# megvii-research/CVPR2023-UniDistill

Hardware: AMD Instinct MI355X
Metric: distill-train samples/sec (nuScenes frame); bev_pool+voxelize HBM GB/s (higher is better)
Workload: dtype f32; 1 GPU; camera_exp_distill_lidar: student+teacher distillation step, 6 cams 256x704, 30000-pt cloud, 40 GT boxes, fwd+bwd+AdamW; batch_per_gpu=4, global_batch=4, parallelism=dp1, layout=channels-last dense convs, executor=eager+DDP, strict_no_library_fallthrough=True, wgrad_stream=on, ranks=1, dist_backend=none (single process)

## Files before the change

cvpr2023-unidistill_amd/csrc/spconv_conv.hip:

```cpp
#include "ud_common.h"
#include "ud_prof.h"
#include "spconv_tile.h"
#include <cstdlib>

namespace {

template <int CIN_P, int COUT_P>
__global__ __launch_bounds__(256) void k_conv_mfma(const float* __restrict__ in, int cin,
                                                   const int32_t* __restrict__ nbr, int K,
                                                   int mirror, const float* __restrict__ W,
                                                   WStrides ws, const float* __restrict__ bias,
                                                   float* __restrict__ out, int cout, int Mout) {
  constexpr int LDA = CIN_P + 4;
  extern __shared__ __attribute__((aligned(16))) char smem[];
  float* As = reinterpret_cast<float*>(smem);
  float* Bs = As + kTM * LDA;
  int* s_nbr = reinterpret_cast<int*>(Bs + COUT_P * LDA);
  const int tid = threadIdx.x, lane = tid & 63, wave = tid >> 6;
  const int g = lane >> 4, li = lane & 15;
  const int row0 = blockIdx.x * kTM;
  constexpr int NT = COUT_P / 16;
  f32x4 acc[NT];
#pragma unroll
  for (int t = 0; t < NT; ++t) acc[t] = (f32x4){0.f, 0.f, 0.f, 0.f};
// ... 57 lines not shown
    __syncthreads();
  }
#pragma unroll
  for (int t = 0; t < NT; ++t) {
    const int col = t * 16 + li;
    if (col >= cout) continue;
    const float bv = bias ? bias[col] : 0.f;
#pragma unroll
    for (int r = 0; r < 4; ++r) {
      const int row = row0 + wave * 16 + 4 * g + r;
      if (row < Mout) out[(size_t)row * cout + col] = acc[t][r] + bv;
    }
  }
}


template <int CIN_P, int COUT_P, bool VA, bool VB>
__global__ __launch_bounds__(512) void k_conv_mfma_v2(const float* __restrict__ in, int cin,
                                                      const int32_t* __restrict__ nbr, int K,
                                                      int mirror, const float* __restrict__ W,
                                                      WStrides ws, const float* __restrict__ bias,
                                                      float* __restrict__ out, int cout, int Mout,
                                                      const int32_t* __restrict__ order,
                                                      ConvEpilogue ep) {
  constexpr int LDA = CIN_P + 8;
  constexpr int NT = COUT_P / 16;
  constexpr int A4 = kTM2 * (CIN_P / 4) / 512;
  constexpr int B4 = (COUT_P * (CIN_P / 4) + 511) / 512;
  constexpr int BU = COUT_P * (CIN_P / 4);
  extern __shared__ __attribute__((aligned(16))) char smem[];
  float* As = reinterpret_cast<float*>(smem);
  float* Bs = As + kTM2 * LDA;
  int* s_nbr = reinterpret_cast<int*>(Bs + COUT_P * LDA);
  unsigned& s_active = *reinterpret_cast<unsigned*>(s_nbr + K * kTM2);
  int* s_row = s_nbr + K * kTM2 + 4;
  const int tid = threadIdx.x, lane = tid & 63, wave = tid >> 6;
  const int g = lane >> 4, li = lane & 15;
  const SpTile tile = sp_tile_setup<16>(s_nbr, s_active, s_row, nbr, K, mirror, order, Mout, tid, lane, wave);
  const unsigned active = tile.active, wmask = tile.wmask;
  f32x4 acc[NT];
#pragma unroll
  for (int t = 0; t < NT; ++t) acc[t] = (f32x4){0.f, 0.f, 0.f, 0.f};
  float4 ra[A4], rb[VB ? B4 : 1];
  constexpr int PER = CIN_P / 4, RPP = 512 / PER;
  const int r0 = tid / PER, c4 = (tid % PER) * 4;
  const bool cok = c4 < cin;
  const float* in_c = in + (cok ? c4 : 0);
  const int wc4 = cok ? c4 : 0;

  auto fetch_a = [&](int k, int j) {
    const int rr = s_nbr[k * kTM2 + r0 + RPP * j];
    if constexpr (VA) {
      ra[j] = *reinterpret_cast<const float4*>(in_c + (size_t)(rr < 0 ? 0 : rr) * cin);
    } else {
      float4 v = make_float4(0.f, 0.f, 0.f, 0.f);
      if (rr >= 0) {
        const float* src = in + (size_t)rr * cin + c4;
        if (c4 + 0 < cin) v.x = src[0];
        if (c4 + 1 < cin) v.y = src[1];
        if (c4 + 2 < cin) v.z = src[2];
        if (c4 + 3 < cin) v.w = src[3];
// ... 108 lines not shown
__global__ __launch_bounds__(512) void k_conv_mfma_bf16(const float* __restrict__ in, int cin,
                                                        const int32_t* __restrict__ nbr, int K,
                                                        int mirror, const float* __restrict__ W,
                                                        WStrides ws, const float* __restrict__ bias,
                                                        float* __restrict__ out, int cout, int Mout,
                                                        const int32_t* __restrict__ order,
                                                        ConvEpilogue ep, int io) {
  const bool in_bf = io & 1, out_bf = io & 2, w_bf = io & 4;
  const unsigned short* in_h = reinterpret_cast<const unsigned short*>(in);
  const unsigned short* W_h = reinterpret_cast<const unsigned short*>(W);
  constexpr int LDB = CIN_P + 8;
  constexpr int NT = COUT_P / 16;
  constexpr int A4 = kTM2 * (CIN_P / 4) / 512;
  constexpr int B4 = (COUT_P * (CIN_P / 4) + 511) / 512;
  constexpr int BU = COUT_P * (CIN_P / 4);
  extern __shared__ __attribute__((aligned(16))) char smem[];
  unsigned short* As = reinterpret_cast<unsigned short*>(smem);
  unsigned short* Bs = As + kTM2 * LDB;
  int* s_nbr = reinterpret_cast<int*>(Bs + COUT_P * LDB);
  unsigned& s_active = *reinterpret_cast<unsigned*>(s_nbr + K * kTM2);
  int* s_row = s_nbr + K * kTM2 + 4;
  const int tid = threadIdx.x, lane = tid & 63, wave = tid >> 6;
  const int g = lane >> 4, li = lane & 15;
  const SpTile tile = sp_tile_setup<16>(s_nbr, s_active, s_row, nbr, K, mirror, order, Mout, tid, lane, wave);
  const unsigned active = tile.active, wmask = tile.wmask;
  f32x4 acc[NT];
#pragma unroll
  for (int t = 0; t < NT; ++t) acc[t] = (f32x4){0.f, 0.f, 0.f, 0.f};
  const bool vecA = (cin & 3) == 0;
  const bool vecB = (ws.sc == 1) && vecA;
  float4 ra[A4];
  auto fetch = [&](int k) {
#pragma unroll
    for (int j = 0; j < A4; ++j) {
      const int u = tid + 512 * j;
      const int row = u / (CIN_P / 4), c4 = (u - row * (CIN_P / 4)) * 4;
      const int rr = s_nbr[k * kTM2 + row];
      float4 v = make_float4(0.f, 0.f, 0.f, 0.f);
      if (rr >= 0 && in_bf) {
        if (c4 < cin) {
          const uint2 h = *reinterpret_cast<const uint2*>(in_h + (size_t)rr * cin + c4);
          v.x = __uint_as_float(h.x);
          v.y = __uint_as_float(h.y);
        }
      } else if (rr >= 0) {
        const float* src = in + (size_t)rr * cin + c4;
        if (vecA) {
// ... 88 lines not shown
  return ((a > o ? a : o) + 15) / 16 * 16;
}

template <int CIN_P, int COUT_P>
__global__ __launch_bounds__(512) void k_conv_mfma_bf16_fast(
    const unsigned short* __restrict__ in, int cin, const int32_t* __restrict__ nbr, int K, int mirror,
    const unsigned short* __restrict__ W, WStrides ws, const float* __restrict__ bias,
    unsigned short* __restrict__ out, int cout, int Mout, const int32_t* __restrict__ order,
    ConvEpilogue ep) {
  constexpr int LDB = CIN_P + 8;
  constexpr int NT = COUT_P / 16;
  constexpr int AU = kTM2 * (CIN_P / 8);
  constexpr int BU = COUT_P * (CIN_P / 8);
  constexpr int A8 = (AU + 511) / 512, B8 = (BU + 511) / 512;
  extern __shared__ __attribute__((aligned(16))) char smem[];
  unsigned short* As = reinterpret_cast<unsigned short*>(smem);
  unsigned short* Bs = As + kTM2 * LDB;
  int* s_nbr = reinterpret_cast<int*>(smem + fast_front_bytes(CIN_P, COUT_P));
  unsigned& s_active = *reinterpret_cast<unsigned*>(s_nbr + K * kTM2);
  int* s_row = s_nbr + K * kTM2 + 4;
  float* Os = reinterpret_cast<float*>(smem);
  const int tid = threadIdx.x, lane = tid & 63, wave = tid >> 6;
  const int g = lane >> 4, li = lane & 15;
  const SpTile tile = sp_tile_setup<16>(s_nbr, s_active, s_row, nbr, K, mirror, order, Mout, tid, lane, wave);
  const unsigned active = tile.active, wmask = tile.wmask;
  f32x4 acc[NT];
#pragma unroll
  for (int t = 0; t < NT; ++t) acc[t] = (f32x4){0.f, 0.f, 0.f, 0.f};
  uint4 ra[A8], rb[B8];
  auto fetch = [&](int k) {
#pragma unroll
    for (int j = 0; j < A8; ++j) {
      const int u = tid + 512 * j;
      ra[j] = make_uint4(0u, 0u, 0u, 0u);
      if (u < AU) {
        const int row = u / (CIN_P / 8), c8 = (u - row * (CIN_P / 8)) * 8;
        const int rr = s_nbr[k * kTM2 + row];
        if (rr >= 0 && c8 < cin) ra[j] = *reinterpret_cast<const uint4*>(in + (size_t)rr * cin + c8);
      }
    }
#pragma unroll
    for (int j = 0; j < B8; ++j) {
      const int u = tid + 512 * j;
      rb[j] = make_uint4(0u, 0u, 0u, 0u);
      if (u < BU) {
        const int n = u / (CIN_P / 8), c8 = (u - n * (CIN_P / 8)) * 8;
        if (n < cout && c8 < cin) rb[j] = *reinterpret_cast<const uint4*>(W + n * ws.sn + k * ws.sk + c8);
// ... 53 lines not shown
  const size_t o = (size_t)kTM2 * (cout_p + 4) * 4;
  return ((a > o ? a : o) + 15) / 16 * 16;
}

template <int CIN_P, int COUT_P>
__global__ __launch_bounds__(512) void k_conv_mfma_bf16_dma(
    const unsigned short* __restrict__ in, int cin, const int32_t* __restrict__ nbr, int K, int mirror,
    const unsigned short* __restrict__ W, WStrides ws, const float* __restrict__ bias,
    unsigned short* __restrict__ out, int cout, int Mout, const int32_t* __restrict__ order,
    ConvEpilogue ep) {
  constexpr int NT = COUT_P / 16;
  constexpr int S = CIN_P / 8;
  constexpr int RPP = 64 / S;
  constexpr int APIECES = kTM2 / RPP, BPIECES = (COUT_P + RPP - 1) / RPP;
  extern __shared__ __attribute__((aligned(16))) char smem[];
  unsigned short* As = reinterpret_cast<unsigned short*>(smem);
  unsigned short* Bs = As + 2 * kTM2 * CIN_P;
  int* s_nbr = reinterpret_cast<int*>(smem + dma_front_bytes(CIN_P, COUT_P));
  unsigned& s_active = *reinterpret_cast<unsigned*>(s_nbr + K * kTM2);
  int* s_row = s_nbr + K * kTM2 + 4;
  float* Os = reinterpret_cast<float*>(smem);
  const int tid = threadIdx.x, lane = tid & 63, wave = tid >> 6;
  const int g = lane >> 4, li = lane & 15;
  const SpTile tile = sp_tile_setup<16>(s_nbr, s_active, s_row, nbr, K, mirror, order, Mout, tid, lane, wave);
  const unsigned active = tile.active, wmask = tile.wmask;
  f32x4 acc[NT];
#pragma unroll
  for (int t = 0; t < NT; ++t) acc[t] = (f32x4){0.f, 0.f, 0.f, 0.f};
  auto swz = [](int r) -> int {
    if (S == 16) return r & 15;
    if (S == 8) return (r >> 1) & 7;
    const int q = (r >> 2) & 3;
    return q == 0 ? 0 : (q == 1 ? 2 : (q == 2 ? 3 : 1));
  };
  const unsigned short* zero = reinterpret_cast<const unsigned short*>(g_sp_zero16);
  const int prow = lane / S, pslot = lane % S;
  auto stage = [&](int k, int buf) {
#pragma unroll
    for (int j = 0; j < (APIECES + 7) / 8; ++j) {
      const int piece = wave + 8 * j;
      if (piece < APIECES) {
        const int r = piece * RPP + prow;
        const int rr = s_nbr[k * kTM2 + r];
        const unsigned short* src = rr >= 0 ? in + (size_t)rr * cin + ((pslot ^ swz(r)) << 3) : zero;
        __builtin_amdgcn_global_load_lds((const __attribute__((address_space(1))) void*)src,
                                         (__attribute__((address_space(3))) void*)(As + (buf * kTM2 + piece * RPP) * CIN_P),
                                         16, 0, 0);
// ... 53 lines not shown
  const long long t = (long long)blockIdx.x * 256 + threadIdx.x;
  if (t >= (long long)Mout * cout) return;
  const int row = (int)(t / cout), n = (int)(t - (long long)row * cout);
  float acc = 0.f;
  for (int k = 0; k < K; ++k) {
    const int r = nbr[(size_t)row * K + (mirror ? K - 1 - k : k)];
    if (r < 0) continue;
    const float* x = in + (size_t)r * cin;
    const float* w = W + n * ws.sn + k * ws.sk;
    for (int c = 0; c < cin; ++c) acc = fmaf(x[c], w[c * ws.sc], acc);
  }
  out[t] = acc + (bias ? bias[n] : 0.f);
}

constexpr unsigned kDmaOob = 0xFFFF0000u;
__device__ __forceinline__ void sp_dma16(__amdgpu_buffer_rsrc_t rsrc, unsigned voff, unsigned soff, unsigned lds_wave_base) {
  __builtin_amdgcn_raw_ptr_buffer_load_lds(rsrc, (__attribute__((address_space(3))) void*)(size_t)lds_wave_base, 16, voff, soff, 0, 0);
}

template <int CIN, int COUT, int NBUF>
__global__ __launch_bounds__(512) void k_conv_dma_f32(const float* __restrict__ in, const int32_t* __restrict__ nbr, int K,
                                                      int mirror, const float* __restrict__ W, WStrides ws,
                                                      const float* __restrict__ bias, float* __restrict__ out, int Mout,
                                                      const int32_t* __restrict__ order, ConvEpilogue ep) {
  constexpr int NT = COUT / 32;
  constexpr int kAB = kTM2 * 256, kWB = COUT * 256, kStage = kAB + kWB;
  constexpr int kHalves = CIN / 64;
  constexpr int kAPieces = kTM2 / 4, kWPieces = COUT / 4;
  extern __shared__ __attribute__((aligned(16))) char smem[];
  int* s_nbr = reinterpret_cast<int*>(smem + NBUF * kStage);
  unsigned& s_active = *reinterpret_cast<unsigned*>(s_nbr + K * kTM2);
  int* s_row = s_nbr + K * kTM2 + 4;
  const int tid = threadIdx.x, lane = tid & 63;
  const int wave = __builtin_amdgcn_readfirstlane(tid >> 6);
  const int g = lane >> 4, li = lane & 15;
  const int wm = wave >> 1, wn = wave & 1;
  const SpTile tile = sp_tile_setup<32>(s_nbr, s_active, s_row, nbr, K, mirror, order, Mout, tid, lane, wm);
  const unsigned active = tile.active, wmask = tile.wmask;
  f32x4 acc[2][NT];
#pragma unroll
  for (int i = 0; i < 2; ++i)
#pragma unroll
    for (int t = 0; t < NT; ++t) acc[i][t] = (f32x4){0.f, 0.f, 0.f, 0.f};

  const __amdgpu_buffer_rsrc_t rin = __builtin_amdgcn_make_buffer_rsrc((void*)in, 0, (int)kDmaOob, 0x00020000);
  const __amdgpu_buffer_rsrc_t rw = __builtin_amdgcn_make_buffer_rsrc((void*)W, 0, (int)kDmaOob, 0x00020000);
  const unsigned swz = (unsigned)((li ^ ((4 * wave + g) & 15)) << 4);
  unsigned wvo[kWPieces / 8];
#pragma unroll
  for (int i = 0; i < kWPieces / 8; ++i) wvo[i] = (unsigned)(4 * (wave + 8 * i) + g) * (unsigned)ws.sn * 4u + swz;
  auto stage = [&](int k, int half, int buf) {
    const unsigned sb = (unsigned)(size_t)smem + buf * kStage;
    int rr[kAPieces / 8];
    {
      const unsigned na = NBUF * kStage + (unsigned)(k * kTM2 + 4 * wave + g) * 4u;
#pragma unroll
      for (int i = 0; i < kAPieces / 8; ++i) asm volatile("ds_read_b32 %0, %1 offset:%2" : "=v"(rr[i]) : "v"(na), "n"(i * 128));
      asm volatile("s_waitcnt lgkmcnt(0)" ::: "memory");
#pragma unroll
      for (int i = 0; i < kAPieces / 8; ++i) asm volatile("" : "+v"(rr[i]));
// ... 82 lines not shown
  for (int t = 0; t < NT; ++t) {
    const int col = wn * (COUT / 2) + t * 16 + li;
    const float bv = bias ? bias[col] : 0.f;
    const float sc = ep.scale ? ep.scale[col] : 1.f;
    const float sh = ep.shift ? ep.shift[col] : 0.f;
#pragma unroll
    for (int i = 0; i < 2; ++i)
#pragma unroll
      for (int r = 0; r < 4; ++r) {
        const int row = s_row[wm * 32 + 16 * i + 4 * g + r];
        if (row >= 0) {
          float v = acc[i][t][r] + bv;
          if (ep.scale) v = v * sc + sh;
          if (ep.residual) v += ep.residual[(size_t)row * COUT + col];
          if (ep.relu) v = fmaxf(v, 0.f);
          out[(size_t)row * COUT + col] = v;
        }
      }
  }
}

template <int CIN, int COUT>
int launch_conv_dma_f32(const float* in, const int32_t* nbr, int K, int mirror, const float* W, WStrides ws,
                        const float* bias, float* out, int Mout, const int32_t* order, ConvEpilogue ep,
                        hipStream_t stream) {
  constexpr int NBUF = 2;
  constexpr size_t front = NBUF * (size_t)(kTM2 * 256 + COUT * 256);
  const size_t lds = front + sp_tile_meta_bytes(K);
  if (lds > kSpLdsMax) return UD_ERR_UNSUPPORTED;
  static UdDeviceOnce attr_set;
  if (const int e = ud_allow_dyn_lds(attr_set, sp_lds_limit(front), k_conv_dma_f32<CIN, COUT, NBUF>)) return e;
  k_conv_dma_f32<CIN, COUT, NBUF><<<ud_div_up(Mout, kTM2), 512, lds, stream>>>(in, nbr, K, mirror, W, ws, bias, out, Mout, order, ep);
  UD_LAUNCH_CHECK();
  return UD_OK;
}

template <int CIN_P, int COUT_P>
int launch_conv_v2(const float* in, int cin, const int32_t* nbr, int K, int mirror, const float* W,
                   WStrides ws, const float* bias, float* out, int cout, int Mout,
                   const int32_t* order, ConvEpilogue ep, hipStream_t stream) {
  constexpr size_t front = (size_t)(kTM2 + COUT_P) * (CIN_P + 8) * sizeof(float);
  const size_t lds = front + sp_tile_meta_bytes(K);
  static UdDeviceOnce attr_set;
  if (const int e = ud_allow_dyn_lds(attr_set, sp_lds_limit(front), k_conv_mfma_v2<CIN_P, COUT_P, true, true>,
                                     k_conv_mfma_v2<CIN_P, COUT_P, true, false>, k_conv_mfma_v2<CIN_P, COUT_P, false, false>))
    return e;
  const bool va = (cin & 3) == 0, vb = va && ws.sc == 1;
  const dim3 grid(ud_div_up(Mout, kTM2));
  if (vb)
    k_conv_mfma_v2<CIN_P, COUT_P, true, true><<<grid, 512, lds, stream>>>(in, cin, nbr, K, mirror, W, ws, bias, out, cout,
                                                                          Mout, order, ep);
  else if (va)
    k_conv_mfma_v2<CIN_P, COUT_P, true, false><<<grid, 512, lds, stream>>>(in, cin, nbr, K, mirror, W, ws, bias, out, cout,
                                                                           Mout, order, ep);
  else
    k_conv_mfma_v2<CIN_P, COUT_P, false, false><<<grid, 512, lds, stream>>>(in, cin, nbr, K, mirror, W, ws, bias, out,
                                                                            cout, Mout, order, ep);
  UD_LAUNCH_CHECK();
  return UD_OK;
}

template <int CIN_P, int COUT_P>
int launch_conv_bf16(const float* in, int cin, const int32_t* nbr, int K, int mirror, const float* W,
                     WStrides ws, const float* bias, float* out, int cout, int Mout,
                     const int32_t* order, ConvEpilogue ep, int io, hipStream_t stream) {
  constexpr int CP = CIN_P < 32 ? 32 : CIN_P;
  if ((io & 1) && (cin & 3)) return UD_ERR_UNSUPPORTED;
  if ((io & 4) && !(ws.sc == 1 && (cin & 3) == 0)) return UD_ERR_UNSUPPORTED;
  if (io == 7 && cin == CP && (cout & 7) == 0 && (ws.sn & 7) == 0 && (ws.sk & 7) == 0) {
    const size_t lds_d = dma_front_bytes(CP, COUT_P) + sp_tile_meta_bytes(K);
    if (lds_d <= kSpLdsMax) {
      static UdDeviceOnce dma_attr_set;
      if (const int e = ud_allow_dyn_lds(dma_attr_set, sp_lds_limit(dma_front_bytes(CP, COUT_P)), k_conv_mfma_bf16_dma<CP, COUT_P>))
        return e;
      k_conv_mfma_bf16_dma<CP, COUT_P><<<ud_div_up(Mout, kTM2), 512, lds_d, stream>>>(
          reinterpret_cast<const unsigned short*>(in), cin, nbr, K, mirror,
          reinterpret_cast<const unsigned short*>(W), ws, bias, reinterpret_cast<unsigned short*>(out), cout,
          Mout, order, ep);
      UD_LAUNCH_CHECK();
      return UD_OK;
// ... 4 lines not shown
    static UdDeviceOnce fast_attr_set;
    if (const int e = ud_allow_dyn_lds(fast_attr_set, sp_lds_limit(fast_front_bytes(CP, COUT_P)), k_conv_mfma_bf16_fast<CP, COUT_P>))
      return e;
    k_conv_mfma_bf16_fast<CP, COUT_P><<<ud_div_up(Mout, kTM2), 512, lds_f, stream>>>(
        reinterpret_cast<const unsigned short*>(in), cin, nbr, K, mirror,
        reinterpret_cast<const unsigned short*>(W), ws, bias, reinterpret_cast<unsigned short*>(out), cout,
        Mout, order, ep);
    UD_LAUNCH_CHECK();
    return UD_OK;
  }
  constexpr size_t front = (size_t)(kTM2 + COUT_P) * (CP + 8) * sizeof(unsigned short);
  const size_t lds = front + sp_tile_meta_bytes(K);
  static UdDeviceOnce attr_set;
  if (const int e = ud_allow_dyn_lds(attr_set, sp_lds_limit(front), k_conv_mfma_bf16<CP, COUT_P>)) return e;
  k_conv_mfma_bf16<CP, COUT_P><<<ud_div_up(Mout, kTM2), 512, lds, stream>>>(
      in, cin, nbr, K, mirror, W, ws, bias, out, cout, Mout, order, ep, io);
  UD_LAUNCH_CHECK();
  return UD_OK;
}

template <int CIN_P, int COUT_P>
int launch_conv(const float* in, int cin, const int32_t* nbr, int K, int mirror, const float* W,
                WStrides ws, const float* bias, float* out, int cout, int Mout,
                const int32_t* order, ConvEpilogue ep, int algo, hipStream_t stream) {
  if (K <= 32 && algo == 3)
    return launch_conv_bf16<CIN_P, COUT_P>(in, cin, nbr, K, mirror, W, ws, bias, out, cout, Mout, order, ep, 0, stream);
  if constexpr ((CIN_P == 64 || CIN_P == 128) && (COUT_P == 64 || COUT_P == 128) && !(CIN_P == 64 && COUT_P == 64)) {
    static const bool no_dma = getenv("UD_SPCONV_NO_DMA") != nullptr;
    const long long w_span = ((long long)(cout - 1) * ws.sn + (long long)(K - 1) * ws.sk + cin) * 4;
    if (!no_dma && K <= 32 && algo == 0 && cin == CIN_P && cout == COUT_P && ws.sc == 1 && (ws.sn & 3) == 0 && (ws.sk & 3) == 0 &&
        ws.sn >= 0 && ws.sk >= 0 && w_span < (long long)kDmaOob && ((size_t)W & 15) == 0 && ((size_t)in & 15) == 0)
      return launch_conv_dma_f32<CIN_P, COUT_P>(in, nbr, K, mirror, W, ws, bias, out, Mout, order, ep, stream);
  }
  if (K <= 32 && algo != 2)
    return launch_conv_v2<CIN_P, COUT_P>(in, cin, nbr, K, mirror, W, ws, bias, out, cout, Mout, order, ep, stream);
  if (ep.scale || ep.residual || ep.relu) return UD_ERR_UNSUPPORTED;
  const size_t lds = (size_t)(kTM + COUT_P) * (CIN_P + 4) * sizeof(float) + kTM * sizeof(int);
  static UdDeviceOnce attr_set;
  if (const int e = ud_allow_dyn_lds(attr_set, (int)lds, k_conv_mfma<CIN_P, COUT_P>)) return e;
  k_conv_mfma<CIN_P, COUT_P><<<ud_div_up(Mout, kTM), 256, lds, stream>>>(
      in, cin, nbr, K, mirror, W, ws, bias, out, cout, Mout);
  UD_LAUNCH_CHECK();
  return UD_OK;
}

}

extern "C" int ud_spconv_conv(const float* in, const int32_t* nbr, const float* W, int64_t w_sn,
                              int64_t w_sk, int64_t w_sc, int mirror, const float* bias,
                              float* out, int Mout, int K, int Cin, int Cout, int algo,
                              const int32_t* row_order, const float* ep_scale,
                              const float* ep_shift, const float* ep_residual, int ep_relu,
                              ud_stream_t stream_) {
  if (Mout < 0 || K <= 0 || Cin <= 0 || Cout <= 0) return UD_ERR_INVALID_ARG;
  if (Mout == 0) return UD_OK;
  if (!in || !nbr || !W || !out) return UD_ERR_INVALID_ARG;
  if ((ep_scale == nullptr) != (ep_shift == nullptr)) return UD_ERR_INVALID_ARG;
  ConvEpilogue ep{ep_scale, ep_shift, ep_residual, ep_relu};
  hipStream_t stream = (hipStream_t)stream_;
  WStrides ws{w_sn, w_sk, w_sc};
  const int cp = pad16(Cin), np = pad16(Cout);
  UdProfScope prof("spconv.k_conv", stream);
  if (algo == 0 || algo == 2 || algo == 3) {
#define X(A, B) \
  if (cp == A && np == B) \
    return launch_conv<A, B>(in, Cin, nbr, K, mirror, W, ws, bias, out, Cout, Mout, row_order, ep, algo, stream);
    UD_CONV_CASES(X)
#undef X
  }
  if (ep.scale || ep.residual || ep.relu) return UD_ERR_UNSUPPORTED;
  k_conv_generic<<<ud_div_up((long long)Mout * Cout, 256), 256, 0, stream>>>(
      in, Cin, nbr, K, mirror, W, ws, bias, out, Cout, Mout);
  UD_LAUNCH_CHECK();
  return UD_OK;
}

extern "C" int ud_spconv_conv_bf16io(const void* in, const int32_t* nbr, const void* W, int64_t w_sn,
                                     int64_t w_sk, int64_t w_sc, int mirror, const float* bias,
                                     void* out, int Mout, int K, int Cin, int Cout, int io_flags,
                                     const int32_t* row_order, const float* ep_scale,
                                     const float* ep_shift, const void* ep_residual, int ep_relu,
                                     ud_stream_t stream_) {
  if (Mout < 0 || K <= 0 || K > 32 || Cin <= 0 || Cout <= 0 || (io_flags & ~7)) return UD_ERR_INVALID_ARG;
  if (Mout == 0) return UD_OK;
  if (!in || !nbr || !W || !out) return UD_ERR_INVALID_ARG;
  if ((ep_scale == nullptr) != (ep_shift == nullptr)) return UD_ERR_INVALID_ARG;
  ConvEpilogue ep{ep_scale, ep_shift, reinterpret_cast<const float*>(ep_residual), ep_relu};
  hipStream_t stream = (hipStream_t)stream_;
  WStrides ws{w_sn, w_sk, w_sc};
// ... 13 lines not shown
```

cvpr2023-unidistill_amd/csrc/spconv_order.hip:

```cpp
#include "ud_common.h"
#include "ud_prof.h"
#include "radix_sort.h"
#include <algorithm>
#include <cstring>

namespace {

__global__ __launch_bounds__(256) void k_offset_counts(const int32_t* __restrict__ nbr, int M, int K, int step,
                                                       unsigned* __restrict__ cnt) {
  __shared__ unsigned s_cnt[32];
  if (threadIdx.x < 32) s_cnt[threadIdx.x] = 0u;
  __syncthreads();
  const long long total = (long long)((M + step - 1) / step) * K;
  for (long long e = (long long)blockIdx.x * 256 + threadIdx.x; e < total; e += (long long)gridDim.x * 256) {
    const int r = (int)(e / K) * step, k = (int)(e % K);
    if (nbr[(size_t)r * K + k] >= 0) atomicAdd(&s_cnt[k], 1u);
  }
  __syncthreads();
  if ((int)threadIdx.x < K && s_cnt[threadIdx.x]) atomicAdd(&cnt[threadIdx.x], s_cnt[threadIdx.x]);
}

__global__ __launch_bounds__(256) void k_row_masks(const int32_t* __restrict__ nbr, int M, int K,
                                                   const unsigned* __restrict__ cnt, unsigned* __restrict__ mask) {
  __shared__ unsigned s_c[32];
// ... 28 lines not shown
};

OrderWs carve_order(void* ws, int M, int K) {
  (void)K;
  UdArena a(ws, (size_t)-1);
  OrderWs w;
  w.nblk = ud_div_up(M, kRsChunk);
  w.cnt = a.take<unsigned>(32);
  w.mask = a.take<unsigned>(M);
  w.keys[0] = a.take<unsigned>(M);
  w.keys[1] = a.take<unsigned>(M);
  w.vals[0] = a.take<int32_t>(M);
  w.vals[1] = a.take<int32_t>(M);
  w.hist = a.take<unsigned>((size_t)kRsBinsMax * w.nblk);
  w.dtot = a.take<unsigned>(kRsBinsMax);
  w.total_bytes = a.used;
  return w;
}

int radix_order(const OrderWs& w, int M, int bits, int32_t* order, hipStream_t stream) {
  return rs_sort_pairs<unsigned>(w.mask, M, bits, order, w.keys, w.vals, w.hist, w.dtot, stream);
}

}

extern "C" size_t ud_spconv_mask_order_workspace_bytes(int M, int K) {
  if (M <= 0 || K <= 0 || K > 31) return 0;
  return carve_order(nullptr, M, K).total_bytes;
}

extern "C" int ud_spconv_mask_order(const int32_t* nbr, int M, int K, int32_t* order, void* workspace, size_t workspace_bytes,
                                    ud_stream_t stream_) {
  if (!nbr || !order || M <= 0 || K <= 0 || K > 31) return UD_ERR_INVALID_ARG;
  if (!workspace || workspace_bytes < ud_spconv_mask_order_workspace_bytes(M, K)) return UD_ERR_WORKSPACE;
  hipStream_t stream = (hipStream_t)stream_;
  OrderWs w = carve_order(workspace, M, K);
  UdProfScope prof("spconv.mask_order", stream);
  const int step = M / 4096 > 1 ? M / 4096 : 1;
  UD_HIP_TRY(hipMemsetAsync(w.cnt, 0, 32 * sizeof(unsigned), stream));
  const long long sampled = (long long)((M + step - 1) / step) * K;
  k_offset_counts<<<(unsigned)std::min<long long>(64, (sampled + 2047) / 2048), 256, 0, stream>>>(nbr, M, K, step, w.cnt);
  UD_LAUNCH_CHECK();
  k_row_masks<<<ud_div_up(M, 256), 256, 0, stream>>>(nbr, M, K, w.cnt, w.mask);
  UD_LAUNCH_CHECK();
  return radix_order(w, M, K, order, stream);
}
```

cvpr2023-unidistill_amd/csrc/spconv_tile.h:

```cpp
#pragma once
#include "ud_common.h"

namespace {

typedef float f32x4 __attribute__((ext_vector_type(4)));
typedef short bf16x8 __attribute__((ext_vector_type(8)));

constexpr int kTM = 64;
constexpr int kTM2 = 128;

struct WStrides {
  long long sn, sk, sc;
};

struct ConvEpilogue {
  const float* scale;
  const float* shift;
  const float* residual;
  int relu;
};

inline int pad16(int c) { return (c + 15) / 16 * 16; }

#define UD_CONV_CASES(X) \
  X(16, 16) X(16, 32) X(32, 16) X(32, 32) X(32, 64) X(64, 32) X(64, 64) X(64, 128) X(128, 64) X(128, 128)

constexpr size_t sp_tile_meta_bytes(int K) { return (size_t)K * kTM2 * sizeof(int) + 16 + kTM2 * sizeof(int); }
constexpr int kSpMaxK = 32;
constexpr size_t kSpLdsMax = 160 * 1024;
constexpr int sp_lds_limit(size_t front) {
  return (int)(front + sp_tile_meta_bytes(kSpMaxK) < kSpLdsMax ? front + sp_tile_meta_bytes(kSpMaxK) : kSpLdsMax);
}

#ifdef __HIPCC__
__device__ __attribute__((aligned(16))) unsigned int g_sp_zero16[4];

__device__ __forceinline__ int sp_next_offset(unsigned todo) { return todo ? (__ffs((int)todo) - 1) : -1; }

struct SpTile {
  int row0;
  unsigned active;
  unsigned wmask;
};

template <int RPW>
__device__ __forceinline__ SpTile sp_tile_setup(int* s_nbr, unsigned& s_active, int* s_row,
                                                const int32_t* nbr, int K, int mirror,
                                                const int32_t* order, int Mout, int tid, int lane,
                                                int wgroup) {
  SpTile t;
  t.row0 = (int)(gridDim.x - 1u - blockIdx.x) * kTM2;
  if (tid == 0) s_active = 0u;
  if (tid < kTM2) {
    const int p = t.row0 + tid;
    s_row[tid] = (p < Mout) ? (order ? order[p] : p) : -1;
  }
  __syncthreads();
  unsigned mine = 0u;
  for (int idx = tid; idx < kTM2 * K; idx += 512) {
    const int r = idx / K, k = idx - r * K;
    int v = -1;
    const int orow = s_row[r];
    if (orow >= 0) v = nbr[(size_t)orow * K + (mirror ? K - 1 - k : k)];
    s_nbr[k * kTM2 + r] = v;
    if (v >= 0) mine |= 1u << k;
  }
#pragma unroll
  for (int o = 32; o > 0; o >>= 1) mine |= __shfl_xor((int)mine, o);
  if (lane == 0 && mine) atomicOr(&s_active, mine);
  __syncthreads();
  t.active = s_active;
  t.wmask = 0u;
  for (int k = 0; k < K; ++k) {
    const int v = (lane < RPW) ? s_nbr[k * kTM2 + wgroup * RPW + lane] : -1;
// ... 80 lines not shown
```

cvpr2023-unidistill_amd/unidistill_amd/ops/spconv.py:

```python
import ctypes
import math

import torch
from torch import nn

from .. import _lib
from . import bn_act


def _triple(v):
    if isinstance(v, (list, tuple)):
        assert len(v) == 3
        return tuple(int(x) for x in v)
    return (int(v),) * 3


def _i3(v):
    return (ctypes.c_int * 3)(*v)


class _SiteSet:

    def __init__(self, indices, spatial_shape, batch_size, rows_sorted):
        self.indices = indices
# ... 125 lines not shown
        return root


_ORDER_CACHE_ATTR = "_ud_mask_order"


def mask_order(nbr, mirror=False):
    key = _ORDER_CACHE_ATTR
    order = getattr(nbr, key, None)
    if order is None:
        K = nbr.shape[1]
        if K > 31 or nbr.shape[0] == 0:
            order = False
        else:
            lib = _lib.load()
            M = nbr.shape[0]
            ws = _lib.workspace(nbr.device, lib.ud_spconv_mask_order_workspace_bytes(M, K), "mask_order")
            order = torch.empty(M, dtype=torch.int32, device=nbr.device)
            _lib.ud.ud_spconv_mask_order(nbr, M, K, order, ws, ws.numel(), _lib.stream_of(nbr))
        setattr(nbr, key, order)
    return None if order is False else order


CONV_LOG = None


def _conv(feat, nbr, weight, w_strides, mirror, bias, cin, cout, algo=0, scale=None, shift=None,
          residual=None, relu=False):
    Mout, K = nbr.shape
    if CONV_LOG is not None:
        CONV_LOG.append((nbr, cin, cout, "f32"))
    out = torch.empty((Mout, cout), dtype=torch.float32, device=feat.device)
    order = mask_order(nbr, mirror) if algo in (0, 3) else None
    if feat.numel() * feat.element_size() >= 0xFFFF0000:
        raise ValueError("ud_spconv_conv: the input feature tensor must be smaller than 4 GiB - 64 KiB (32-bit byte offsets)")
    _lib.ud.ud_spconv_conv(feat, nbr, weight, w_strides[0], w_strides[1], w_strides[2], 1 if mirror else 0, bias, out, Mout, K,
                           cin, cout, algo, order, scale, shift, residual, 1 if relu else 0, _lib.stream_of(feat))
    return out


def tile_masks(nbr):
    hit = getattr(nbr, "_ud_tile_masks", None)
    if hit is None:
        Mout, K = nbr.shape
        hit = torch.empty(((Mout + 63) // 64,), dtype=torch.int32, device=nbr.device)
        _lib.ud.ud_spconv_tile_masks(nbr, Mout, K, mask_order(nbr, False), hit, _lib.stream_of(nbr))
        nbr._ud_tile_masks = hit
    return hit


def sorted_rulebook(nbr):
    hit = getattr(nbr, "_ud_sorted", None)
    if hit is None:
        order = mask_order(nbr, False)
        hit = nbr if order is None else nbr.index_select(0, order.long()).contiguous()
        nbr._ud_sorted = hit
    return hit


def _conv_bf16io(feat, nbr, weight, bias, cin, cout, scale=None, shift=None, residual=None, relu=False,
# ... 65 lines not shown
        return 3
    return algo


class _SparseConvFn(torch.autograd.Function):

    @staticmethod
    def forward(ctx, features, weight, bias, nbr, nbr_t, mirror_t, algo):
        _lib.require_gpu(features, weight, nbr)
        cout, cin = weight.shape[0], weight.shape[-1]
        K = nbr.shape[1]
        assert weight.numel() == cout * K * cin and features.shape[1] == cin
        algo = effective_algo(algo)
        b32 = None if bias is None else bias.detach().contiguous().float()
        if algo == 3 and K <= 32 and cin % 8 == 0 and cout % 8 == 0:
            xb = features.detach().to(torch.bfloat16).contiguous()
            wb = weight.detach().reshape(cout, K, cin).to(torch.bfloat16).contiguous()
            out = _conv_bf16io(xb, nbr, wb, b32, cin, cout)
            ctx.save_for_backward(xb, wb, nbr, nbr_t)
            ctx.cfg = (mirror_t, "bf16io", bias is not None, weight.shape, features.dtype)
            return out
        features = features.contiguous().float()
        w = weight.contiguous().float()
        out = _conv(features, nbr, w, (K * cin, cin, 1), False, b32, cin, cout, algo)
        ctx.save_for_backward(features, w, nbr, nbr_t)
        ctx.cfg = (mirror_t, algo, bias is not None, weight.shape, torch.float32)
        return out

    @staticmethod
    def backward(ctx, gout):
        features, w, nbr, nbr_t = ctx.saved_tensors
        mirror_t, algo, has_bias, wshape, in_dtype = ctx.cfg
        cout, cin = wshape[0], wshape[-1]
        K = nbr.shape[1]
        lib = _lib.load()
        Mout = nbr.shape[0]
        gin = gw = gb = None
        if algo == "bf16io":
            gout = gout.to(torch.bfloat16).contiguous()
            if ctx.needs_input_grad[0]:
                wt = w.permute(2, 1, 0).contiguous()
                gin = _conv_bf16io(gout, nbr_t, wt, None, cout, cin, mirror=mirror_t).to(in_dtype)
            if ctx.needs_input_grad[1]:
                gw = torch.empty(wshape, dtype=torch.float32, device=w.device)
                need = lib.ud_spconv_wgrad_bf16_workspace_bytes(Mout, K, cin, cout)
                ws = _lib.workspace(w.device, need, "spconv_wgrad")
                order = mask_order(nbr, False)
# ... 227 lines not shown
        out_sites, nbr, nbr_t, mirror = self._rulebooks(x)
        feats = _SparseConvFn.apply(x.features, self.weight, self.bias, nbr, nbr_t, mirror,
                                    self.kernel_algo)
        return SparseConvTensor(feats, None, None, None, _sites=out_sites, _indice_dict=x.indice_dict)

    def forward_fused(self, x, bn=None, relu=False, residual=None):
        out_sites, nbr, _, _ = self._rulebooks(x)
        w = self.weight.detach().contiguous().float()
        cout, cin = w.shape[0], w.shape[-1]
        K = nbr.shape[1]
        scale = shift = None
        if bn is not None:
            scale, shift = folded_batchnorm(bn)
        with torch.no_grad():
            bias = None if self.bias is None else self.bias.detach().contiguous().float()
            if effective_algo(0) == 3 and K <= 32:
                feats = _conv_bf16io(x.features.detach().contiguous(), nbr,
                                     bf16_weight(self) if cin % 4 == 0 else w.view(cout, K, cin), bias, cin,
                                     cout, scale, shift,
                                     None if residual is None else residual.detach().contiguous(), relu)
            else:
                feats = _conv(x.features.detach().contiguous().float(), nbr, w, (K * cin, cin, 1), False,
                              bias, cin, cout, 0, scale, shift,
                              None if residual is None else residual.detach().contiguous().float(), relu)
        return SparseConvTensor(feats, None, None, None, _sites=out_sites, _indice_dict=x.indice_dict)


class SubMConv3d(_SparseConvBase):
    def __init__(self, in_channels, out_channels, kernel_size, stride=1, padding=0, dilation=1,
                 groups=1, bias=True, indice_key=None, algo=None, **kw):
        super().__init__(in_channels, out_channels, kernel_size, stride, padding, dilation, groups,
                         bias, subm=True, indice_key=indice_key, algo=algo)


class SparseConv3d(_SparseConvBase):
    def __init__(self, in_channels, out_channels, kernel_size, stride=1, padding=0, dilation=1,
                 groups=1, bias=True, indice_key=None, algo=None, **kw):
        super().__init__(in_channels, out_channels, kernel_size, stride, padding, dilation, groups,
                         bias, subm=False, indice_key=indice_key, algo=algo)


class SparseInverseConv3d(_SparseConvBase):
    def __init__(self, in_channels, out_channels, kernel_size, indice_key=None, bias=True,
                 algo=None, **kw):
        super().__init__(in_channels, out_channels, kernel_size, 1, 0, 1, 1, bias, subm=False,
                         inverse=True, indice_key=indice_key, algo=algo)

# ... 6 lines not shown
```

include/unidistill_hip.h:

```cpp
#ifndef UNIDISTILL_HIP_H
#define UNIDISTILL_HIP_H

#include <stddef.h>
#include <stdint.h>

#ifdef __cplusplus
extern "C" {
#endif

typedef void* ud_stream_t;

#define UD_OK 0
#define UD_ERR_INVALID_ARG (-1)
#define UD_ERR_WORKSPACE (-2)
#define UD_ERR_HIP (-3)
#define UD_ERR_UNSUPPORTED (-4)

const char* ud_version(void);
int ud_abi_version(void);
const char* ud_error_string(int code);

void ud_prof_enable(int on);
int ud_prof_read(const char* name, double* total_ms, int* calls, int reset);

// ... 62 lines not shown

int ud_spconv_subm_rulebook(const void* index, int rows_sorted, const int32_t* coords, int M,
                            int B, int Dz, int Hy, int Wx, int kz, int ky, int kx, int32_t* nbr,
                            ud_stream_t stream);

int ud_spconv_down_outputs(const int32_t* in_coords, int Min, int B, int Dz, int Hy, int Wx,
                           const int* ksize, const int* stride, const int* pad, void* out_index,
                           size_t out_index_bytes, int32_t* out_coords, int out_cap,
                           int32_t* m_out, ud_stream_t stream);
int ud_spconv_build_index_dev(const int32_t* coords, const int32_t* m_dev, int M_cap, int B, int Dz, int Hy, int Wx,
                              int rows_sorted, void* index, size_t index_bytes, ud_stream_t stream);
int ud_spconv_down_outputs_dev(const int32_t* in_coords, const int32_t* min_dev, int Min_cap, int B, int Dz, int Hy,
                               int Wx, const int* ksize, const int* stride, const int* pad, void* out_index,
                               size_t out_index_bytes, int32_t* out_coords, int out_cap, int32_t* m_out,
                               ud_stream_t stream);

int ud_spconv_down_rulebook(const void* in_index, int in_rows_sorted, int Min, int B, int Dz,
                            int Hy, int Wx, const int* ksize, const int* stride, const int* pad,
                            const int32_t* out_coords, int Mout, int32_t* out_nbr,
                            int32_t* in_nbr, ud_stream_t stream);

int ud_spconv_conv(const float* in, const int32_t* nbr, const float* W, int64_t w_sn, int64_t w_sk,
                   int64_t w_sc, int mirror, const float* bias, float* out, int Mout, int K,
                   int Cin, int Cout, int algo, const int32_t* row_order, const float* ep_scale,
                   const float* ep_shift, const float* ep_residual, int ep_relu, ud_stream_t stream);

size_t ud_spconv_wgrad_bf16_workspace_bytes(int Mout, int K, int Cin, int Cout);
int ud_spconv_wgrad_bf16(const void* in, const int32_t* nbr, const void* gout, float* gW, int Mout,
                         int K, int Cin, int Cout, int io_bf16, const int32_t* row_order,
                         const unsigned* tile_masks, void* workspace, size_t workspace_bytes,
                         ud_stream_t stream);
int ud_spconv_tile_masks(const int32_t* nbr, int Mout, int K, const int32_t* row_order, unsigned* masks,
                         ud_stream_t stream);
size_t ud_spconv_mask_order_workspace_bytes(int Mout, int K);
int ud_spconv_mask_order(const int32_t* nbr, int Mout, int K, int32_t* order, void* workspace, size_t workspace_bytes,
                         ud_stream_t stream);
int ud_spconv_conv_bf16io(const void* in, const int32_t* nbr, const void* W, int64_t w_sn,
                          int64_t w_sk, int64_t w_sc, int mirror, const float* bias, void* out,
                          int Mout, int K, int Cin, int Cout, int io_flags, const int32_t* row_order,
                          const float* ep_scale, const float* ep_shift, const void* ep_residual,
                          int ep_relu, ud_stream_t stream);
size_t ud_spconv_wgrad_workspace_bytes(int Mout, int K, int Cin, int Cout);
int ud_spconv_wgrad(const float* in, const int32_t* nbr, const float* gout, float* gW, int Mout,
                    int K, int Cin, int Cout, int algo, void* workspace, size_t workspace_bytes,
                    ud_stream_t stream);

int ud_sparse_to_dense(const float* feat, const int32_t* coords, int M, int C, int B, int Dz,
                       int Hy, int Wx, float* dense, void* workspace, size_t workspace_bytes,
                       ud_stream_t stream);
int ud_dense_to_sparse(const float* gdense, const int32_t* coords, int M, int C, int B, int Dz,
                       int Hy, int Wx, float* gfeat, void* workspace, size_t workspace_bytes,
                       ud_stream_t stream);
size_t ud_sparse_bev_workspace_bytes(int B, int Dz, int Hy, int Wx);
int ud_sparse_to_bev_bf16(const void* feat, const int32_t* coords, int M, int C, int B, int Dz, int Hy,
                          int Wx, void* bev, void* workspace, size_t workspace_bytes, ud_stream_t stream);
int ud_bev_to_sparse_bf16(const void* gbev, const int32_t* coords, int M, int C, int B, int Dz, int Hy,
                          int Wx, void* gfeat, void* workspace, size_t workspace_bytes, ud_stream_t stream);
int ud_sparse_to_bev_f32(const float* feat, const int32_t* coords, int M, int C, int B, int Dz, int Hy, int Wx, float* bev,
                         void* workspace, size_t workspace_bytes, ud_stream_t stream);
// ... 464 lines not shown
```

Measured before the change: 68.96 samples/s.

## Schedule sparse-conv tiles heaviest-first via a per-tile cost permutation

Adds a kernel that computes, per 128-row tile of the mask-ordered rulebook, how many of the K kernel offsets are active, then radix-sorts the tiles so those with the most active offsets come first. Forward f32 submanifold convs with K=27 and cin>=64 pass this permutation to the MFMA and DMA conv kernels, which read their tile index from it instead of using reversed block order. The aim is to reduce tail imbalance by launching expensive tiles early. The cost is an extra kernel and sort per rulebook (cached on the nbr tensor) and an indirect tile lookup.

```diff
diff --git a/cvpr2023-unidistill_amd/csrc/spconv_conv.hip b/cvpr2023-unidistill_amd/csrc/spconv_conv.hip
--- a/cvpr2023-unidistill_amd/csrc/spconv_conv.hip
+++ b/cvpr2023-unidistill_amd/csrc/spconv_conv.hip
@@ -103,6 +103,7 @@
                                                       WStrides ws, const float* __restrict__ bias,
                                                       float* __restrict__ out, int cout, int Mout,
                                                       const int32_t* __restrict__ order,
+                                                      const int32_t* __restrict__ tile_perm,
                                                       ConvEpilogue ep) {
   constexpr int LDA = CIN_P + 8;
   constexpr int NT = COUT_P / 16;
@@ -117,7 +118,7 @@
   int* s_row = s_nbr + K * kTM2 + 4;
   const int tid = threadIdx.x, lane = tid & 63, wave = tid >> 6;
   const int g = lane >> 4, li = lane & 15;
-  const SpTile tile = sp_tile_setup<16>(s_nbr, s_active, s_row, nbr, K, mirror, order, Mout, tid, lane, wave);
+  const SpTile tile = sp_tile_setup<16>(s_nbr, s_active, s_row, nbr, K, mirror, order, Mout, tid, lane, wave, sp_tile_index(tile_perm));
   const unsigned active = tile.active, wmask = tile.wmask;
   f32x4 acc[NT];
 #pragma unroll
@@ -272,7 +273,7 @@
   int* s_row = s_nbr + K * kTM2 + 4;
   const int tid = threadIdx.x, lane = tid & 63, wave = tid >> 6;
   const int g = lane >> 4, li = lane & 15;
-  const SpTile tile = sp_tile_setup<16>(s_nbr, s_active, s_row, nbr, K, mirror, order, Mout, tid, lane, wave);
+  const SpTile tile = sp_tile_setup<16>(s_nbr, s_active, s_row, nbr, K, mirror, order, Mout, tid, lane, wave, sp_tile_index(nullptr));
   const unsigned active = tile.active, wmask = tile.wmask;
   f32x4 acc[NT];
 #pragma unroll
@@ -407,7 +408,7 @@
   float* Os = reinterpret_cast<float*>(smem);
   const int tid = threadIdx.x, lane = tid & 63, wave = tid >> 6;
   const int g = lane >> 4, li = lane & 15;
-  const SpTile tile = sp_tile_setup<16>(s_nbr, s_active, s_row, nbr, K, mirror, order, Mout, tid, lane, wave);
+  const SpTile tile = sp_tile_setup<16>(s_nbr, s_active, s_row, nbr, K, mirror, order, Mout, tid, lane, wave, sp_tile_index(nullptr));
   const unsigned active = tile.active, wmask = tile.wmask;
   f32x4 acc[NT];
 #pragma unroll
@@ -507,7 +508,7 @@
   float* Os = reinterpret_cast<float*>(smem);
   const int tid = threadIdx.x, lane = tid & 63, wave = tid >> 6;
   const int g = lane >> 4, li = lane & 15;
-  const SpTile tile = sp_tile_setup<16>(s_nbr, s_active, s_row, nbr, K, mirror, order, Mout, tid, lane, wave);
+  const SpTile tile = sp_tile_setup<16>(s_nbr, s_active, s_row, nbr, K, mirror, order, Mout, tid, lane, wave, sp_tile_index(nullptr));
   const unsigned active = tile.active, wmask = tile.wmask;
   f32x4 acc[NT];
 #pragma unroll
@@ -607,7 +608,8 @@
 __global__ __launch_bounds__(512) void k_conv_dma_f32(const float* __restrict__ in, const int32_t* __restrict__ nbr, int K,
                                                       int mirror, const float* __restrict__ W, WStrides ws,
                                                       const float* __restrict__ bias, float* __restrict__ out, int Mout,
-                                                      const int32_t* __restrict__ order, ConvEpilogue ep) {
+                                                      const int32_t* __restrict__ order,
+                                                      const int32_t* __restrict__ tile_perm, ConvEpilogue ep) {
   constexpr int NT = COUT / 32;
   constexpr int kAB = kTM2 * 256, kWB = COUT * 256, kStage = kAB + kWB;
   constexpr int kHalves = CIN / 64;
@@ -620,7 +622,7 @@
   const int wave = __builtin_amdgcn_readfirstlane(tid >> 6);
   const int g = lane >> 4, li = lane & 15;
   const int wm = wave >> 1, wn = wave & 1;
-  const SpTile tile = sp_tile_setup<32>(s_nbr, s_active, s_row, nbr, K, mirror, order, Mout, tid, lane, wm);
+  const SpTile tile = sp_tile_setup<32>(s_nbr, s_active, s_row, nbr, K, mirror, order, Mout, tid, lane, wm, sp_tile_index(tile_perm));
   const unsigned active = tile.active, wmask = tile.wmask;
   f32x4 acc[2][NT];
 #pragma unroll
@@ -749,15 +751,15 @@
 
 template <int CIN, int COUT>
 int launch_conv_dma_f32(const float* in, const int32_t* nbr, int K, int mirror, const float* W, WStrides ws,
-                        const float* bias, float* out, int Mout, const int32_t* order, ConvEpilogue ep,
-                        hipStream_t stream) {
+                        const float* bias, float* out, int Mout, const int32_t* order, const int32_t* tile_perm,
+                        ConvEpilogue ep, hipStream_t stream) {
   constexpr int NBUF = 2;
   constexpr size_t front = NBUF * (size_t)(kTM2 * 256 + COUT * 256);
   const size_t lds = front + sp_tile_meta_bytes(K);
   if (lds > kSpLdsMax) return UD_ERR_UNSUPPORTED;
   static UdDeviceOnce attr_set;
   if (const int e = ud_allow_dyn_lds(attr_set, sp_lds_limit(front), k_conv_dma_f32<CIN, COUT, NBUF>)) return e;
-  k_conv_dma_f32<CIN, COUT, NBUF><<<ud_div_up(Mout, kTM2), 512, lds, stream>>>(in, nbr, K, mirror, W, ws, bias, out, Mout, order, ep);
+  k_conv_dma_f32<CIN, COUT, NBUF><<<ud_div_up(Mout, kTM2), 512, lds, stream>>>(in, nbr, K, mirror, W, ws, bias, out, Mout, order, tile_perm, ep);
   UD_LAUNCH_CHECK();
   return UD_OK;
 }
@@ -765,7 +767,7 @@
 template <int CIN_P, int COUT_P>
 int launch_conv_v2(const float* in, int cin, const int32_t* nbr, int K, int mirror, const float* W,
                    WStrides ws, const float* bias, float* out, int cout, int Mout,
-                   const int32_t* order, ConvEpilogue ep, hipStream_t stream) {
+                   const int32_t* order, const int32_t* tile_perm, ConvEpilogue ep, hipStream_t stream) {
   constexpr size_t front = (size_t)(kTM2 + COUT_P) * (CIN_P + 8) * sizeof(float);
   const size_t lds = front + sp_tile_meta_bytes(K);
   static UdDeviceOnce attr_set;
@@ -776,13 +778,13 @@
   const dim3 grid(ud_div_up(Mout, kTM2));
   if (vb)
     k_conv_mfma_v2<CIN_P, COUT_P, true, true><<<grid, 512, lds, stream>>>(in, cin, nbr, K, mirror, W, ws, bias, out, cout,
-                                                                          Mout, order, ep);
+                                                                          Mout, order, tile_perm, ep);
   else if (va)
     k_conv_mfma_v2<CIN_P, COUT_P, true, false><<<grid, 512, lds, stream>>>(in, cin, nbr, K, mirror, W, ws, bias, out, cout,
-                                                                           Mout, order, ep);
+                                                                           Mout, order, tile_perm, ep);
   else
     k_conv_mfma_v2<CIN_P, COUT_P, false, false><<<grid, 512, lds, stream>>>(in, cin, nbr, K, mirror, W, ws, bias, out,
-                                                                            cout, Mout, order, ep);
+                                                                            cout, Mout, order, tile_perm, ep);
   UD_LAUNCH_CHECK();
   return UD_OK;
 }
@@ -833,7 +835,7 @@
 template <int CIN_P, int COUT_P>
 int launch_conv(const float* in, int cin, const int32_t* nbr, int K, int mirror, const float* W,
                 WStrides ws, const float* bias, float* out, int cout, int Mout,
-                const int32_t* order, ConvEpilogue ep, int algo, hipStream_t stream) {
+                const int32_t* order, const int32_t* tile_perm, ConvEpilogue ep, int algo, hipStream_t stream) {
   if (K <= 32 && algo == 3)
     return launch_conv_bf16<CIN_P, COUT_P>(in, cin, nbr, K, mirror, W, ws, bias, out, cout, Mout, order, ep, 0, stream);
   if constexpr ((CIN_P == 64 || CIN_P == 128) && (COUT_P == 64 || COUT_P == 128) && !(CIN_P == 64 && COUT_P == 64)) {
@@ -841,10 +843,10 @@
     const long long w_span = ((long long)(cout - 1) * ws.sn + (long long)(K - 1) * ws.sk + cin) * 4;
     if (!no_dma && K <= 32 && algo == 0 && cin == CIN_P && cout == COUT_P && ws.sc == 1 && (ws.sn & 3) == 0 && (ws.sk & 3) == 0 &&
         ws.sn >= 0 && ws.sk >= 0 && w_span < (long long)kDmaOob && ((size_t)W & 15) == 0 && ((size_t)in & 15) == 0)
-      return launch_conv_dma_f32<CIN_P, COUT_P>(in, nbr, K, mirror, W, ws, bias, out, Mout, order, ep, stream);
+      return launch_conv_dma_f32<CIN_P, COUT_P>(in, nbr, K, mirror, W, ws, bias, out, Mout, order, tile_perm, ep, stream);
   }
   if (K <= 32 && algo != 2)
-    return launch_conv_v2<CIN_P, COUT_P>(in, cin, nbr, K, mirror, W, ws, bias, out, cout, Mout, order, ep, stream);
+    return launch_conv_v2<CIN_P, COUT_P>(in, cin, nbr, K, mirror, W, ws, bias, out, cout, Mout, order, tile_perm, ep, stream);
   if (ep.scale || ep.residual || ep.relu) return UD_ERR_UNSUPPORTED;
   const size_t lds = (size_t)(kTM + COUT_P) * (CIN_P + 4) * sizeof(float) + kTM * sizeof(int);
   static UdDeviceOnce attr_set;
@@ -860,7 +862,7 @@
 extern "C" int ud_spconv_conv(const float* in, const int32_t* nbr, const float* W, int64_t w_sn,
                               int64_t w_sk, int64_t w_sc, int mirror, const float* bias,
                               float* out, int Mout, int K, int Cin, int Cout, int algo,
-                              const int32_t* row_order, const float* ep_scale,
+                              const int32_t* row_order, const int32_t* tile_perm, const float* ep_scale,
                               const float* ep_shift, const float* ep_residual, int ep_relu,
                               ud_stream_t stream_) {
   if (Mout < 0 || K <= 0 || Cin <= 0 || Cout <= 0) return UD_ERR_INVALID_ARG;
@@ -875,7 +877,7 @@
   if (algo == 0 || algo == 2 || algo == 3) {
 #define X(A, B) \
   if (cp == A && np == B) \
-    return launch_conv<A, B>(in, Cin, nbr, K, mirror, W, ws, bias, out, Cout, Mout, row_order, ep, algo, stream);
+    return launch_conv<A, B>(in, Cin, nbr, K, mirror, W, ws, bias, out, Cout, Mout, row_order, tile_perm, ep, algo, stream);
     UD_CONV_CASES(X)
 #undef X
   }
diff --git a/cvpr2023-unidistill_amd/csrc/spconv_order.hip b/cvpr2023-unidistill_amd/csrc/spconv_order.hip
--- a/cvpr2023-unidistill_amd/csrc/spconv_order.hip
+++ b/cvpr2023-unidistill_amd/csrc/spconv_order.hip
@@ -74,6 +74,48 @@
   return rs_sort_pairs<unsigned>(w.mask, M, bits, order, w.keys, w.vals, w.hist, w.dtot, stream);
 }
 
+constexpr int kTileRows = 128;
+constexpr int kTileKeyBits = 5;
+
+__global__ __launch_bounds__(kTileRows) void k_tile_costs(const int32_t* __restrict__ nbr, int M, int K,
+                                                          const int32_t* __restrict__ order,
+                                                          int32_t* __restrict__ cost, unsigned* __restrict__ key) {
+  __shared__ unsigned s_m[kTileRows / 64];
+  const int t = blockIdx.x, p = t * kTileRows + (int)threadIdx.x;
+  unsigned m = 0u;
+  if (p < M) {
+    const int32_t* row = nbr + (size_t)(order ? order[p] : p) * K;
+#pragma unroll 9
+    for (int k = 0; k < K; ++k) m |= (unsigned)(row[k] >= 0) << k;
+  }
+#pragma unroll
+  for (int o = 32; o > 0; o >>= 1) m |= (unsigned)__shfl_xor((int)m, o);
+  if ((threadIdx.x & 63) == 0) s_m[threadIdx.x >> 6] = m;
+  __syncthreads();
+  if (threadIdx.x == 0) {
+    const int c = __popc(s_m[0] | s_m[1]);
+    cost[t] = c;
+    key[t] = (unsigned)(K - c);
+  }
+}
+
+struct TilePermWs {
+  unsigned* key;
+  unsigned* hist;
+  unsigned* dtot;
+  size_t total_bytes;
+};
+
+TilePermWs carve_tile_perm(void* ws, int T) {
+  UdArena a(ws, (size_t)-1);
+  TilePermWs w;
+  w.key = a.take<unsigned>(T);
+  w.hist = a.take<unsigned>((size_t)kRsBinsMax * ud_div_up(T, kRsChunk));
+  w.dtot = a.take<unsigned>(kRsBinsMax);
+  w.total_bytes = a.used;
+  return w;
+}
+
 }
 
 extern "C" size_t ud_spconv_mask_order_workspace_bytes(int M, int K) {
@@ -97,3 +139,25 @@
   UD_LAUNCH_CHECK();
   return radix_order(w, M, K, order, stream);
 }
+
+extern "C" size_t ud_spconv_tile_perm_workspace_bytes(int M, int K) {
+  if (M <= 0 || K <= 0 || K > 31) return 0;
+  return carve_tile_perm(nullptr, ud_div_up(M, kTileRows)).total_bytes;
+}
+
+extern "C" int ud_spconv_tile_perm(const int32_t* nbr, int M, int K, const int32_t* row_order, int32_t* tile_cost,
+                                   int32_t* tile_perm, void* workspace, size_t workspace_bytes, ud_stream_t stream_) {
+  if (!nbr || !tile_cost || !tile_perm || M <= 0 || K <= 0 || K > 31) return UD_ERR_INVALID_ARG;
+  if (!workspace || workspace_bytes < ud_spconv_tile_perm_workspace_bytes(M, K)) return UD_ERR_WORKSPACE;
+  hipStream_t stream = (hipStream_t)stream_;
+  const int T = ud_div_up(M, kTileRows);
+  TilePermWs w = carve_tile_perm(workspace, T);
+  UdProfScope prof("spconv.tile_perm", stream);
+  static_assert(kTileRows == 128, "k_tile_costs combines two waves");
+  k_tile_costs<<<T, kTileRows, 0, stream>>>(nbr, M, K, row_order, tile_cost, w.key);
+  UD_LAUNCH_CHECK();
+  unsigned* const ktmp[2] = {nullptr, nullptr};
+  int32_t* const vtmp[2] = {nullptr, nullptr};
+  static_assert(kTileKeyBits <= 9, "one radix pass");
+  return rs_sort_pairs<unsigned>(w.key, T, kTileKeyBits, tile_perm, ktmp, vtmp, w.hist, w.dtot, stream);
+}
diff --git a/cvpr2023-unidistill_amd/csrc/spconv_tile.h b/cvpr2023-unidistill_amd/csrc/spconv_tile.h
--- a/cvpr2023-unidistill_amd/csrc/spconv_tile.h
+++ b/cvpr2023-unidistill_amd/csrc/spconv_tile.h
@@ -43,13 +43,17 @@
   unsigned wmask;
 };
 
+__device__ __forceinline__ int sp_tile_index(const int32_t* tile_perm) {
+  return tile_perm ? __builtin_amdgcn_readfirstlane(tile_perm[blockIdx.x]) : (int)(gridDim.x - 1u - blockIdx.x);
+}
+
 template <int RPW>
 __device__ __forceinline__ SpTile sp_tile_setup(int* s_nbr, unsigned& s_active, int* s_row,
                                                 const int32_t* nbr, int K, int mirror,
                                                 const int32_t* order, int Mout, int tid, int lane,
-                                                int wgroup) {
+                                                int wgroup, int tile_index) {
   SpTile t;
-  t.row0 = (int)(gridDim.x - 1u - blockIdx.x) * kTM2;
+  t.row0 = tile_index * kTM2;
   if (tid == 0) s_active = 0u;
   if (tid < kTM2) {
     const int p = t.row0 + tid;
diff --git a/cvpr2023-unidistill_amd/unidistill_amd/ops/spconv.py b/cvpr2023-unidistill_amd/unidistill_amd/ops/spconv.py
--- a/cvpr2023-unidistill_amd/unidistill_amd/ops/spconv.py
+++ b/cvpr2023-unidistill_amd/unidistill_amd/ops/spconv.py
@@ -1,5 +1,6 @@
 import ctypes
 import math
+import os
 
 import torch
 from torch import nn
@@ -171,20 +172,43 @@
     return None if order is False else order
 
 
+def tile_perm(nbr):
+    hit = getattr(nbr, "_ud_tile_perm", None)
+    if hit is None:
+        order = mask_order(nbr, False)
+        if order is None:
+            hit = False
+        else:
+            lib = _lib.load()
+            M, K = nbr.shape
+            T = (M + 127) // 128
+            ws = _lib.workspace(nbr.device, lib.ud_spconv_tile_perm_workspace_bytes(M, K), "tile_perm")
+            hit = (torch.empty(T, dtype=torch.int32, device=nbr.device), torch.empty(T, dtype=torch.int32, device=nbr.device))
+            _lib.ud.ud_spconv_tile_perm(nbr, M, K, order, hit[0], hit[1], ws, ws.numel(), _lib.stream_of(nbr))
+        nbr._ud_tile_perm = hit
+    return None if hit is False else hit
+
+
 CONV_LOG = None
+TILE_PERM_LOG = None
 
 
 def _conv(feat, nbr, weight, w_strides, mirror, bias, cin, cout, algo=0, scale=None, shift=None,
-          residual=None, relu=False):
+          residual=None, relu=False, forward=False):
     Mout, K = nbr.shape
     if CONV_LOG is not None:
         CONV_LOG.append((nbr, cin, cout, "f32"))
     out = torch.empty((Mout, cout), dtype=torch.float32, device=feat.device)
     order = mask_order(nbr, mirror) if algo in (0, 3) else None
+    perm = None
+    if forward and algo == 0 and K == 27 and cin >= 64 and order is not None and not os.environ.get("UD_SPCONV_NO_TILE_PERM"):
+        perm = tile_perm(nbr)[1]
+    if TILE_PERM_LOG is not None:
+        TILE_PERM_LOG.append((nbr, cin, cout, perm is not None))
     if feat.numel() * feat.element_size() >= 0xFFFF0000:
         raise ValueError("ud_spconv_conv: the input feature tensor must be smaller than 4 GiB - 64 KiB (32-bit byte offsets)")
     _lib.ud.ud_spconv_conv(feat, nbr, weight, w_strides[0], w_strides[1], w_strides[2], 1 if mirror else 0, bias, out, Mout, K,
-                           cin, cout, algo, order, scale, shift, residual, 1 if relu else 0, _lib.stream_of(feat))
+                           cin, cout, algo, order, perm, scale, shift, residual, 1 if relu else 0, _lib.stream_of(feat))
     return out
 
 
@@ -296,7 +320,7 @@
             return out
         features = features.contiguous().float()
         w = weight.contiguous().float()
-        out = _conv(features, nbr, w, (K * cin, cin, 1), False, b32, cin, cout, algo)
+        out = _conv(features, nbr, w, (K * cin, cin, 1), False, b32, cin, cout, algo, forward=True)
         ctx.save_for_backward(features, w, nbr, nbr_t)
         ctx.cfg = (mirror_t, algo, bias is not None, weight.shape, torch.float32)
         return out
@@ -570,7 +594,7 @@
             else:
                 feats = _conv(x.features.detach().contiguous().float(), nbr, w, (K * cin, cin, 1), False,
                               bias, cin, cout, 0, scale, shift,
-                              None if residual is None else residual.detach().contiguous().float(), relu)
+                              None if residual is None else residual.detach().contiguous().float(), relu, forward=True)
         return SparseConvTensor(feats, None, None, None, _sites=out_sites, _indice_dict=x.indice_dict)
 
 
diff --git a/include/unidistill_hip.h b/include/unidistill_hip.h
--- a/include/unidistill_hip.h
+++ b/include/unidistill_hip.h
@@ -108,8 +108,9 @@
 
 int ud_spconv_conv(const float* in, const int32_t* nbr, const float* W, int64_t w_sn, int64_t w_sk,
                    int64_t w_sc, int mirror, const float* bias, float* out, int Mout, int K,
-                   int Cin, int Cout, int algo, const int32_t* row_order, const float* ep_scale,
-                   const float* ep_shift, const float* ep_residual, int ep_relu, ud_stream_t stream);
+                   int Cin, int Cout, int algo, const int32_t* row_order, const int32_t* tile_perm,
+                   const float* ep_scale, const float* ep_shift, const float* ep_residual, int ep_relu,
+                   ud_stream_t stream);
 
 size_t ud_spconv_wgrad_bf16_workspace_bytes(int Mout, int K, int Cin, int Cout);
 int ud_spconv_wgrad_bf16(const void* in, const int32_t* nbr, const void* gout, float* gW, int Mout,
@@ -121,6 +122,9 @@
 size_t ud_spconv_mask_order_workspace_bytes(int Mout, int K);
 int ud_spconv_mask_order(const int32_t* nbr, int Mout, int K, int32_t* order, void* workspace, size_t workspace_bytes,
                          ud_stream_t stream);
+size_t ud_spconv_tile_perm_workspace_bytes(int Mout, int K);
+int ud_spconv_tile_perm(const int32_t* nbr, int Mout, int K, const int32_t* row_order, int32_t* tile_cost, int32_t* tile_perm,
+                        void* workspace, size_t workspace_bytes, ud_stream_t stream);
 int ud_spconv_conv_bf16io(const void* in, const int32_t* nbr, const void* W, int64_t w_sn,
                           int64_t w_sk, int64_t w_sc, int mirror, const float* bias, void* out,
                           int Mout, int K, int Cin, int Cout, int io_flags, const int32_t* row_order,
```

Result: no change. 69.22 samples/s (median of 4 runs) (+0.4%).
